# eora-ai/torchok

Measured on AMD Instinct MI355X. Metric: images/sec (node) ResNet-50 224px bs256/GPU; step p50 ms, higher is better.
Workload: dtype bf16

## Files before the change

### include/tok.h

```cpp
#ifndef TOK_H_
#define TOK_H_

#include <stddef.h>
#include <stdint.h>

#ifdef __cplusplus
extern "C" {
#endif

typedef enum tok_status {
  TOK_OK = 0,
  TOK_ERR_INVALID = -1,
  TOK_ERR_LAUNCH = -2,
  TOK_ERR_WORKSPACE = -3
} tok_status;

typedef enum tok_dtype { TOK_F32 = 0, TOK_F16 = 1, TOK_BF16 = 2 } tok_dtype;

typedef struct tok_conv_desc {
  int32_t n, h, w, c;
  int32_t k;
  int32_t r, s;
  int32_t p, q;
  int32_t stride, pad;
// ... 18 lines not shown

typedef struct tok_pack_item {
  const float* src;
  void* dst_fwd;
  void* dst_dgrad;
  int32_t k, r, s, c, k_pad, s_pad, c_pad;
  int32_t block_start;
} tok_pack_item;
int tok_pack_item_blocks(const tok_pack_item* item );
int tok_pack_weights_batched(const tok_pack_item* items_dev, int n_items, int total_blocks, void* stream);


int tok_conv_fwd_stat_rows(const tok_conv_desc* d);
int tok_conv_fwd(const tok_conv_desc* d, const void* x, const void* w, const float* bias,
                 void* y, float* stats, void* stream);
int tok_conv_dgrad(const tok_conv_desc* d, const void* dy, const void* w_dgrad, void* dx,
                   int accumulate, void* stream);
int tok_conv_dgrad_stat_rows(const tok_conv_desc* d);
int tok_conv_dgrad_bnstats(const tok_conv_desc* d, const void* dy, const void* w_dgrad, void* dx,
                           int accumulate, const void* bn_y, const uint8_t* bn_mask, float* partial,
                           void* stream);
typedef struct tok_bn_fused {
  int32_t* counters;
  int64_t count;
  int32_t c_real;
  int32_t param_accumulate;
  float momentum, eps;
  const float* gamma;
  const float* beta;
  float* running_mean;
  float* running_var;
  int64_t* nbt;
  float* mean;
  float* rstd;
  float* scale;
  float* shift;
  float* dgamma;
  float* dbeta;
  float* coef;
} tok_bn_fused;
int tok_conv_fwd_bn(const tok_conv_desc* d, const void* x, const void* w_fwd, void* y, float* stats,
                    const tok_bn_fused* bn, void* stream);
int tok_conv_dgrad_bn(const tok_conv_desc* d, const void* dy, const void* w_dgrad, void* dx, int accumulate,
                      const void* bn_y, const uint8_t* bn_mask, float* partial, const tok_bn_fused* bn,
                      void* stream);
int tok_bn_gram_finalize(const float* Z, const float* zsum, const float* w, int64_t count, int p, int k,
                         const float* gamma, const float* beta, float* running_mean, float* running_var,
                         int64_t* num_batches_tracked, float momentum, float eps, float* mean, float* rstd,
                         float* scale, float* shift, float* wz ,
                         void* stream);
int tok_conv_fwd_bn_apply(const tok_conv_desc* d, const void* x, const void* w, const float* scale, const float* shift,
                          const void* shortcut , int relu, void* out, uint8_t* mask ,
                          void* stream);
int tok_conv_dgrad_maskstore(const tok_conv_desc* d, const void* dy, const void* w_dgrad, void* dx, int accumulate,
                             const uint8_t* mask, float* partial, void* stream);
int tok_relu_mask_reduce(const void* dout, const uint8_t* mask, int64_t m, int c, void* dz, float* partial, void* stream);
int tok_bn3_bwd_prepare(const float* G, const float* w, const float* wz, const float* zsum, const float* partial, int rows,
                        int64_t count, int p, int k, const float* gamma, const float* mean, const float* rstd,
                        float* dgamma, float* dbeta, int param_accumulate, float* coef, float* dw, int dw_accumulate,
                        void* wa, void* wb, float* cvec, float* ws ,
                        void* stream);
size_t tok_bn3_bwd_prepare_ws_floats(int p, int k);
int tok_conv_dgrad_bias(const tok_conv_desc* d, const void* dy, const void* w_dgrad, const float* bias, void* dx,
                        int accumulate, const void* bn_y, const uint8_t* bn_mask, float* partial, void* stream);
int tok_subsample2_fwd(const void* x, int n, int h, int w, int c, void* out, void* stream);
int tok_subsample2_bwd(const void* dsub, int n, int h, int w, int c, void* dx, int accumulate, void* stream);
int tok_conv_dgrad_subacc_ok(const tok_conv_desc* d);
int tok_conv_dgrad_subacc(const tok_conv_desc* d, const void* dy, const void* w_dgrad, void* dx, const void* dsub,
                          const void* bn_y , const uint8_t* mask ,
                          float* partial , int mask_store, void* stream);
int tok_conv_dgrad2_ok(const tok_conv_desc* d1, const tok_conv_desc* d2);
int tok_conv_dgrad2(const tok_conv_desc* d1, const void* dy1, const void* w1_dgrad, const tok_conv_desc* d2, const void* dy2,
                    const void* w2_dgrad, const float* bias , void* dx, int accumulate,
                    const void* bn_y , const uint8_t* bn_mask , float* partial ,
                    void* stream);
size_t tok_conv_wgrad_ws_bytes(const tok_conv_desc* d);
int tok_conv_wgrad(const tok_conv_desc* d, const void* x, const void* dy, float* dw,
                   int k_real, int c_real, void* ws, size_t ws_bytes, int accumulate,
                   void* stream);
int tok_conv_wgrad_bias_ok(const tok_conv_desc* d);
size_t tok_conv_wgrad_bias_ws_bytes(const tok_conv_desc* d);
int tok_conv_wgrad_bias(const tok_conv_desc* d, const void* x, const void* dy, float* dw, int k_real, int c_real,
                        void* ws, size_t ws_bytes, int accumulate, float* dbias, int bias_accumulate, void* stream);


int tok_bn_finalize(const float* stats, int rows, int64_t count, int c, int c_real,
                    const float* gamma, const float* beta,
                    float* running_mean, float* running_var, int64_t* nbt,
                    float momentum, float eps,
                    float* mean, float* rstd, float* scale, float* shift, void* stream);
int tok_bn_eval_coeffs(const float* gamma, const float* beta, const float* running_mean,
                       const float* running_var, float eps, int c, int c_real,
                       float* scale, float* shift, void* stream);
int tok_bn_stats_rows(int64_t m, int c);
int tok_bn_stats(const void* y, int64_t m, int c, float* stats, void* stream);
int tok_bn_act_fwd(const void* y, const float* scale, const float* shift,
                   const void* shortcut, int relu, void* out, uint8_t* mask, int64_t m, int c,
                   void* stream);
void* tok_event_create(void);
int tok_event_destroy(void* ev);
int tok_next_launch_event(void* ev);
int tok_stream_wait_event(void* stream, void* ev);
int tok_bn_act_fwd_colsum_rows(int64_t m, int c);
int tok_bn_act_fwd_colsum(const void* y, const float* scale, const float* shift, const void* shortcut, int relu, void* out,
                          uint8_t* mask, int64_t m, int c, float* partial, void* stream);
int tok_bn_bwd_rows(int64_t m, int c);
int tok_bn_bwd_reduce(const void* dout, const void* y, const uint8_t* mask,
                      const float* scale, const float* shift,
                      const float* mean, const float* rstd, int relu,
                      int64_t m, int c, float* partial, void* stream);
int tok_bn_bwd_finalize(const float* partial, int rows, int64_t m, int c, int c_real,
                        const float* gamma, const float* mean, const float* rstd,
                        float* dgamma, float* dbeta, float* coef, int accumulate, int dzy_form,
                        void* stream);
int tok_bn_bwd_apply(const void* dout, const void* y, const uint8_t* mask,
                     const float* scale, const float* shift, const float* coef, int relu,
                     void* dy, void* dshortcut, int dshortcut_accumulate,
                     int64_t m, int c, void* stream);


int tok_maxpool3x3s2_fwd(const void* x, void* y, uint8_t* argmax, int n, int h, int w, int c,
                         void* stream);
int tok_maxpool3x3s2_bwd(const void* dy, const uint8_t* argmax, void* dx, int accumulate,
                         int n, int h, int w, int c, void* stream);
int tok_avgpool2x2_fwd(const void* x, void* y, int n, int h, int w, int c, void* stream);
int tok_avgpool2x2_bwd(const void* dy, void* dx, int accumulate, int n, int h, int w, int c, void* stream);
int tok_gap_fwd(const void* x, void* y, int n, int hw, int c, void* stream);
int tok_gap_bwd(const void* dy, void* dx, int accumulate, int n, int hw, int c, void* stream);
int tok_global_pool_fwd(const void* x, void* y, int* argmax, int n, int hw, int c, int ldy, int mode, void* stream);
int tok_global_pool_bwd(const void* dy, const int* argmax, void* dx, int accumulate, int n, int hw, int c, int ldy,
                        int mode, void* stream);

int tok_colsum(const void* dy, int64_t m, int n_pad, int n_real, float* out, int accumulate,
               void* stream);

#define TOK_CE_LOSS_FLOATS 2050
int tok_softmax_ce_fwd(const void* logits, const int64_t* target, int rows, int classes, int ld,
                       int64_t ignore_index, float* lse, float* row_loss,
                       float* loss , void* stream);
int tok_softmax_ce_bwd(const void* logits, const int64_t* target, const float* lse,
                       const float* loss, const float* gscale, int rows, int classes, int ld,
                       int64_t ignore_index, void* dlogits, void* stream);

int tok_softmax_ce_smooth_fwd(const void* logits, const int64_t* target, int rows, int classes, int ld,
                              int64_t ignore_index, float label_smoothing, float* lse, float* row_loss,
                              float* loss, void* stream);
int tok_softmax_ce_smooth_bwd(const void* logits, const int64_t* target, const float* lse, const float* loss,
                              const float* gscale, int rows, int classes, int ld, int64_t ignore_index,
                              float label_smoothing, void* dlogits, void* stream);

int tok_upsample_ce_serves(int classes, int ld);
int tok_upsample_ce_fwd(const void* low, int n, int hs, int ws, int classes, int ld, int hd, int wd, const int64_t* target,
                        int64_t ignore_index, float* lse, float* row_loss, float* loss, void* stream);
int tok_upsample_ce_bwd(const void* low, int n, int hs, int ws, int classes, int ld, int hd, int wd, const int64_t* target,
                        int64_t ignore_index, const float* lse, const float* loss, const float* gscale, void* dlow,
                        int accumulate, void* stream);

int tok_dice_rows(int64_t rows);
int tok_dice_fwd(const void* logits, const void* target, int64_t rows, int classes, int ld, int mode, float smooth,
                 float eps, int log_loss, const int64_t* class_sel, int n_sel, float* partial, float* loss,
                 float* coef, void* stream);
int tok_dice_bwd(const void* logits, const void* target, const float* coef, const float* gscale, int64_t rows,
                 int classes, int ld, int mode, void* dlogits, void* stream);

int tok_bce_logits_fwd(const void* logits, const float* target, int64_t rows, int classes, int ld,
                       float ignore_value, int mean, float* loss, void* stream);
// ... 215 lines not shown
```

### torchok_amd/_C.py

```python
import ctypes
import os
from ctypes import POINTER, Structure, c_char_p, c_float, c_int, c_int32, c_int64, c_size_t, c_void_p

_HERE = os.path.dirname(os.path.abspath(__file__))
LIB_PATH = os.environ.get('TOK_LIB') or os.path.join(_HERE, 'lib', 'libtok_gfx950.so')

TOK_F32, TOK_F16, TOK_BF16 = 0, 1, 2
TOK_CE_LOSS_FLOATS = 2050


class ConvDesc(Structure):
    _fields_ = [('n', c_int32), ('h', c_int32), ('w', c_int32), ('c', c_int32),
                ('k', c_int32), ('r', c_int32), ('s', c_int32),
                ('p', c_int32), ('q', c_int32),
                ('stride', c_int32), ('pad', c_int32), ('s_pad', c_int32)]


class PackItem(Structure):
    _fields_ = [('src', c_void_p), ('dst_fwd', c_void_p), ('dst_dgrad', c_void_p),
                ('k', c_int32), ('r', c_int32), ('s', c_int32), ('c', c_int32),
                ('k_pad', c_int32), ('s_pad', c_int32), ('c_pad', c_int32), ('block_start', c_int32)]


class BnFused(Structure):
    _fields_ = [('counters', c_void_p), ('count', c_int64), ('c_real', c_int32), ('param_accumulate', c_int32),
                ('momentum', c_float), ('eps', c_float), ('gamma', c_void_p), ('beta', c_void_p),
                ('running_mean', c_void_p), ('running_var', c_void_p), ('nbt', c_void_p), ('mean', c_void_p),
                ('rstd', c_void_p), ('scale', c_void_p), ('shift', c_void_p), ('dgamma', c_void_p),
                ('dbeta', c_void_p), ('coef', c_void_p)]


TOK_GRAD_CLIP_MAX_PARTIALS = 1024

_P = c_void_p
_PD = POINTER(ConvDesc)

PROTOTYPES = {
    'tok_last_error': (c_char_p, []),
    'tok_version': (c_int, []),
    'tok_nchw_to_nhwc_bf16': (c_int, [_P, c_int, c_int, c_int, c_int, c_int, _P, c_int, _P]),
    'tok_cast_f32_bf16': (c_int, [_P, _P, c_size_t, _P]),
    'tok_cast_bf16_f32': (c_int, [_P, _P, c_float, c_size_t, _P]),
    'tok_pack_weight_fwd': (c_int, [_P, c_int, c_int, c_int, c_int, _P, c_int, c_int, c_int, _P]),
    'tok_pack_weight_dgrad': (c_int, [_P, c_int, c_int, c_int, c_int, _P, c_int, c_int, _P]),
    'tok_pack_weight_both': (c_int, [_P, c_int, c_int, c_int, c_int, _P, c_int, c_int, c_int, _P, _P]),
    'tok_pack_item_blocks': (c_int, [POINTER(PackItem)]),
    'tok_pack_weights_batched': (c_int, [_P, c_int, c_int, _P]),
    'tok_conv_fwd_stat_rows': (c_int, [_PD]),
    'tok_conv_fwd': (c_int, [_PD, _P, _P, _P, _P, _P, _P]),
    'tok_conv_dgrad': (c_int, [_PD, _P, _P, _P, c_int, _P]),
    'tok_conv_dgrad_stat_rows': (c_int, [_PD]),
    'tok_conv_dgrad_bnstats': (c_int, [_PD, _P, _P, _P, c_int, _P, _P, _P, _P]),
    'tok_conv_fwd_bn': (c_int, [_PD, _P, _P, _P, _P, POINTER(BnFused), _P]),
    'tok_conv_dgrad_bn': (c_int, [_PD, _P, _P, _P, c_int, _P, _P, _P, POINTER(BnFused), _P]),
    'tok_conv_wgrad_ws_bytes': (c_size_t, [_PD]),
    'tok_conv_wgrad': (c_int, [_PD, _P, _P, _P, c_int, c_int, _P, c_size_t, c_int, _P]),
    'tok_conv_wgrad_bias_ok': (c_int, [_PD]),
    'tok_conv_wgrad_bias_ws_bytes': (c_size_t, [_PD]),
    'tok_conv_wgrad_bias': (c_int, [_PD, _P, _P, _P, c_int, c_int, _P, c_size_t, c_int, _P, c_int, _P]),
    'tok_bn_finalize': (c_int, [_P, c_int, c_int64, c_int, c_int, _P, _P, _P, _P, _P, c_float, c_float,
                                _P, _P, _P, _P, _P]),
    'tok_bn_eval_coeffs': (c_int, [_P, _P, _P, _P, c_float, c_int, c_int, _P, _P, _P]),
    'tok_bn_stats_rows': (c_int, [c_int64, c_int]),
    'tok_bn_stats': (c_int, [_P, c_int64, c_int, _P, _P]),
    'tok_bn_act_fwd': (c_int, [_P, _P, _P, _P, c_int, _P, _P, c_int64, c_int, _P]),
    'tok_bn_act_fwd_colsum_rows': (c_int, [c_int64, c_int]),
    'tok_event_create': (_P, []),
    'tok_event_destroy': (c_int, [_P]),
    'tok_next_launch_event': (c_int, [_P]),
    'tok_stream_wait_event': (c_int, [_P, _P]),
    'tok_bn_act_fwd_colsum': (c_int, [_P, _P, _P, _P, c_int, _P, _P, c_int64, c_int, _P, _P]),
    'tok_bn_bwd_rows': (c_int, [c_int64, c_int]),
    'tok_bn_bwd_reduce': (c_int, [_P, _P, _P, _P, _P, _P, _P, c_int, c_int64, c_int, _P, _P]),
    'tok_bn_bwd_finalize': (c_int, [_P, c_int, c_int64, c_int, c_int, _P, _P, _P, _P, _P, _P, c_int, c_int, _P]),
    'tok_bn_bwd_apply': (c_int, [_P, _P, _P, _P, _P, _P, c_int, _P, _P, c_int, c_int64, c_int, _P]),
    'tok_maxpool3x3s2_fwd': (c_int, [_P, _P, _P, c_int, c_int, c_int, c_int, _P]),
    'tok_maxpool3x3s2_bwd': (c_int, [_P, _P, _P, c_int, c_int, c_int, c_int, c_int, _P]),
    'tok_avgpool2x2_fwd': (c_int, [_P, _P, c_int, c_int, c_int, c_int, _P]),
    'tok_avgpool2x2_bwd': (c_int, [_P, _P, c_int, c_int, c_int, c_int, c_int, _P]),
    'tok_gap_fwd': (c_int, [_P, _P, c_int, c_int, c_int, _P]),
    'tok_gap_bwd': (c_int, [_P, _P, c_int, c_int, c_int, c_int, _P]),
    'tok_global_pool_fwd': (c_int, [_P, _P, _P, c_int, c_int, c_int, c_int, c_int, _P]),
    'tok_global_pool_bwd': (c_int, [_P, _P, _P, c_int, c_int, c_int, c_int, c_int, c_int, _P]),
    'tok_colsum': (c_int, [_P, c_int64, c_int, c_int, _P, c_int, _P]),
    'tok_bn_gram_finalize': (c_int, [_P, _P, _P, c_int64, c_int, c_int, _P, _P, _P, _P, _P, c_float, c_float, _P, _P, _P, _P, _P, _P]),
    'tok_conv_fwd_bn_apply': (c_int, [POINTER(ConvDesc), _P, _P, _P, _P, _P, c_int, _P, _P, _P]),
    'tok_conv_dgrad_maskstore': (c_int, [POINTER(ConvDesc), _P, _P, _P, c_int, _P, _P, _P]),
    'tok_relu_mask_reduce': (c_int, [_P, _P, c_int64, c_int, _P, _P, _P]),
    'tok_bn3_bwd_prepare': (c_int, [_P, _P, _P, _P, _P, c_int, c_int64, c_int, c_int, _P, _P, _P, _P, _P, c_int, _P, _P, c_int,
                                    _P, _P, _P, _P, _P]),
    'tok_bn3_bwd_prepare_ws_floats': (c_size_t, [c_int, c_int]),
    'tok_conv_dgrad_bias': (c_int, [POINTER(ConvDesc), _P, _P, _P, _P, c_int, _P, _P, _P, _P]),
    'tok_conv_dgrad2_ok': (c_int, [POINTER(ConvDesc), POINTER(ConvDesc)]),
    'tok_conv_dgrad2': (c_int, [POINTER(ConvDesc), _P, _P, POINTER(ConvDesc), _P, _P, _P, _P, c_int, _P, _P, _P, _P]),
    'tok_subsample2_fwd': (c_int, [_P, c_int, c_int, c_int, c_int, _P, _P]),
    'tok_subsample2_bwd': (c_int, [_P, c_int, c_int, c_int, c_int, _P, c_int, _P]),
    'tok_conv_dgrad_subacc_ok': (c_int, [POINTER(ConvDesc)]),
    'tok_conv_dgrad_subacc': (c_int, [POINTER(ConvDesc), _P, _P, _P, _P, _P, _P, _P, c_int, _P]),
    'tok_softmax_ce_fwd': (c_int, [_P, _P, c_int, c_int, c_int, c_int64, _P, _P, _P, _P]),
    'tok_softmax_ce_bwd': (c_int, [_P, _P, _P, _P, _P, c_int, c_int, c_int, c_int64, _P, _P]),
    'tok_softmax_ce_smooth_fwd': (c_int, [_P, _P, c_int, c_int, c_int, c_int64, c_float, _P, _P, _P, _P]),
    'tok_softmax_ce_smooth_bwd': (c_int, [_P, _P, _P, _P, _P, c_int, c_int, c_int, c_int64, c_float, _P, _P]),
    'tok_upsample_ce_serves': (c_int, [c_int, c_int]),
    'tok_upsample_ce_fwd': (c_int, [_P, c_int, c_int, c_int, c_int, c_int, c_int, c_int, _P, c_int64, _P, _P, _P, _P]),
    'tok_upsample_ce_bwd': (c_int, [_P, c_int, c_int, c_int, c_int, c_int, c_int, c_int, _P, c_int64, _P, _P, _P, _P, c_int, _P]),
    'tok_dice_rows': (c_int, [c_int64]),
    'tok_dice_fwd': (c_int, [_P, _P, c_int64, c_int, c_int, c_int, c_float, c_float, c_int, _P, c_int, _P, _P, _P, _P]),
    'tok_dice_bwd': (c_int, [_P, _P, _P, _P, c_int64, c_int, c_int, c_int, _P, _P]),
    'tok_bce_logits_fwd': (c_int, [_P, _P, c_int64, c_int, c_int, c_float, c_int, _P, _P]),
    'tok_bce_logits_bwd': (c_int, [_P, _P, _P, _P, c_int64, c_int, c_int, c_float, c_int, _P, _P]),
    'tok_relevance_matrix_multilabel': (c_int, [_P, _P, c_int, c_int, c_int, _P, _P]),
    'tok_embed_reg_fwd': (c_int, [_P, c_int, c_int, c_int, c_int, _P, _P, _P]),
    'tok_embed_reg_bwd': (c_int, [_P, _P, _P, c_float, c_int, c_int, c_int, c_int, _P, _P]),
    'tok_regression_loss_fwd': (c_int, [_P, _P, c_int64, c_int, c_float, c_int, _P, _P]),
    'tok_regression_loss_bwd': (c_int, [_P, _P, _P, c_int64, c_int, c_float, c_int, _P, _P]),
    'tok_confusion_update': (c_int, [_P, _P, _P, c_int64, c_int, c_int, c_int64, _P, _P]),
    'tok_cls_stats_update': (c_int, [_P, _P, _P, c_int64, c_int, c_int, c_int64, _P, _P]),
    'tok_l2norm_fwd': (c_int, [_P, _P, _P, c_int, c_int, c_int, c_int, c_float, _P]),
    'tok_l2norm_bwd': (c_int, [_P, _P, _P, _P, c_int, c_int, c_int, c_int, c_int, _P]),
    'tok_arcface_margin_fwd': (c_int, [_P, _P, c_int, c_int, c_int, c_float, c_float, c_float, c_float, c_int, c_float, _P, _P]),
    'tok_arcface_margin_bwd': (c_int, [_P, _P, _P, c_int, c_int, c_int, c_float, c_float, c_float, c_float, c_int, c_float, _P, _P]),
    'tok_relevance_matrix': (c_int, [_P, _P, c_int, c_int, _P, _P]),
    'tok_contrastive_fwd': (c_int, [_P, _P, _P, c_int, c_int, c_int, c_int, c_float, _P, _P, _P, _P]),
    'tok_contrastive_bwd': (c_int, [_P, _P, _P, _P, _P, c_int, c_int, c_int, c_int, c_float, _P, _P, c_int, _P]),
    'tok_fuse_sum_relu_fwd': (c_int, [_P, c_int, _P, c_int, _P, c_int, _P, c_int, c_int, c_int, c_int, c_int, c_int, _P, _P, _P]),
    'tok_fuse_sum_affine_relu_fwd': (c_int, [_P, c_int, _P, _P, _P, c_int, _P, _P, _P, c_int, _P, _P, _P, c_int, _P, _P, c_int, c_int, c_int, c_int, c_int, _P, _P, _P]),
    'tok_fuse_sum_relu_bwd': (c_int, [_P, _P, c_int, c_int, c_int, c_int, c_int, _P, c_int, _P]),
    'tok_bilinear_fwd': (c_int, [_P, c_int, c_int, c_int, c_int, c_int, _P, c_int, c_int, c_int, c_int, _P]),
    'tok_bilinear_bwd': (c_int, [_P, c_int, c_int, c_int, c_int, c_int, _P, c_int, c_int, c_int, c_int, c_int, _P]),
    'tok_bilinear_bwd_multi': (c_int, [_P, c_int, c_int, c_int, c_int, _P, c_int, c_int, _P, c_int, c_int, _P, c_int, c_int, _P]),
    'tok_bilinear_sum_stats_rows': (c_int, [c_int, c_int, c_int, c_int]),
    'tok_bilinear_sum_stats': (c_int, [_P, _P, c_int, c_int, _P, c_int, c_int, _P, c_int, c_int, c_int, c_int, c_int, c_int, _P, _P, _P]),
    'tok_layernorm_fwd': (c_int, [_P, _P, _P, c_int, _P, _P, _P, _P, _P, c_int64, c_int, c_int, c_float, _P]),
    'tok_layernorm_bwd_rows': (c_int, [c_int64, c_int]),
    'tok_layernorm_bwd': (c_int, [_P, _P, _P, _P, _P, _P, c_int, _P, c_int, _P, c_int64, c_int, c_int, _P]),
    'tok_colsum_partial_rows': (c_int, [c_int64, c_int]),
    'tok_colsum_partial': (c_int, [_P, c_int64, c_int, _P, _P]),
    'tok_colsum_f32': (c_int, [_P, c_int64, c_int, _P, c_int, _P]),
    'tok_colsum_f32_pair': (c_int, [_P, _P, c_int64, c_int, _P, c_int, _P, c_int, _P]),
    'tok_act_fwd': (c_int, [c_int, _P, _P, c_size_t, _P]),
    'tok_act_bwd': (c_int, [c_int, _P, _P, _P, c_int, c_size_t, _P]),
    'tok_window_attn_fwd': (c_int, [_P, c_int, c_int, c_int, c_int, c_int, c_int, c_int, c_int, _P, _P, _P, _P, _P, _P]),
# ... 105 lines not shown
```

### torchok_amd/csrc/bn.hip

```cpp
#include "tok_common.h"
#include <hip/hip_ext.h>
#include <stdlib.h>

static thread_local hipEvent_t t_done_event = nullptr;

namespace {

struct Geo {
  int cg_total, cge, rpb;
};
inline Geo make_geo(int c) {
  Geo g;
  g.cg_total = c / 8;
  g.cge = g.cg_total < 256 ? g.cg_total : 256;
  g.rpb = 256 / g.cge;
  return g;
}
inline int stream_blocks(int64_t m, const Geo& g, int cap) {
  int64_t b = (m + g.rpb - 1) / g.rpb;
  if (b > cap) b = cap;
  if (b < 1) b = 1;
  return (int)b;
}

// ... 250 lines not shown
        if (relu && mask != nullptr) {
          const unsigned bits = mask[(size_t)m * cg_total + cg];
#pragma unroll
          for (int e = 0; e < 8; ++e) {
            const float yf = bf2f(v[e]);
            const float dz = ((bits >> e) & 1u) ? bf2f(g[e]) : 0.f;
            s1[e] += dz;
            s2[e] = fmaf(dz, (yf - mu[e]) * rs[e], s2[e]);
          }
        } else {
#pragma unroll
          for (int e = 0; e < 8; ++e) {
            const float yf = bf2f(v[e]);
            float dz = bf2f(g[e]);
            if (relu && !(fmaf(yf, sc[e], sh[e]) > 0.f)) dz = 0.f;
            s1[e] += dz;
            s2[e] = fmaf(dz, (yf - mu[e]) * rs[e], s2[e]);
          }
        }
      }
    }
#pragma unroll
    for (int e = 0; e < 8; ++e) { red[0][tid][e] = s1[e]; red[1][tid][e] = s2[e]; }
    __syncthreads();
    if (rl == 0) {
      for (int r = 1; r < rpb; ++r)
#pragma unroll
        for (int e = 0; e < 8; ++e) { s1[e] += red[0][r * cge + cgl][e]; s2[e] += red[1][r * cge + cgl][e]; }
#pragma unroll
      for (int e = 0; e < 8; ++e) {
        partial[((size_t)0 * gridDim.x + blockIdx.x) * C + cg * 8 + e] = s1[e];
        partial[((size_t)1 * gridDim.x + blockIdx.x) * C + cg * 8 + e] = s2[e];
      }
    }
    __syncthreads();
  }
}

template <int CW>
__global__ __launch_bounds__(256) void bn_bwd_finalize_kernel(
    const float* __restrict__ partial, int rows, double inv_m, int C, int Creal, const float* __restrict__ gamma,
    const float* __restrict__ mean, const float* __restrict__ rstd, float* dgamma, float* dbeta,
    float* coef, int accumulate, int dzy_form) {
  __shared__ double red[2][256];
  constexpr int RL = 256 / CW;
  const int tid = threadIdx.x;
  const int cl = tid % CW, rl = tid / CW;
  const int c = blockIdx.x * CW + cl;
  double a1 = 0.0, a2 = 0.0;
  const bool owner = rl == 0 && c < Creal;
  float g_c = 0.f, mu_c = 0.f, rs_c = 0.f, dg_c = 0.f, db_c = 0.f;
  if (owner) {
    g_c = gamma[c]; mu_c = mean[c]; rs_c = rstd[c];
    if (accumulate && dgamma != nullptr) dg_c = dgamma[c];
    if (accumulate && dbeta != nullptr) db_c = dbeta[c];
  }
  if (c < C) {
    fold_rows<RL>(partial, rows, C, c, rl, a1, a2);
  }
  red[0][tid] = a1;
  red[1][tid] = a2;
  __syncthreads();
  for (int s = RL / 2; s > 0; s >>= 1) {
    if (rl < s) {
      red[0][tid] += red[0][tid + s * CW];
      red[1][tid] += red[1][tid + s * CW];
    }
    __syncthreads();
  }
  if (rl == 0 && c >= Creal && c < C) {
    coef[c] = 0.f; coef[C + c] = 0.f; coef[2 * C + c] = 0.f;
  }
  if (owner) {
    float sdz, sdzx, c1, c2, c3;
    bn_bwd_coeffs(red[0][tid], red[1][tid], dzy_form, inv_m, g_c, mu_c, rs_c, sdz, sdzx, c1, c2, c3);
    if (dgamma != nullptr) dgamma[c] = accumulate ? dg_c + sdzx : sdzx;
    if (dbeta != nullptr) dbeta[c] = accumulate ? db_c + sdz : sdz;
    coef[c] = c1;
    coef[C + c] = c2;
    coef[2 * C + c] = c3;
  }
}

__global__ __launch_bounds__(256) void bn_bwd_apply_kernel(
    const bf16* dout, const bf16* __restrict__ y, const uint8_t* __restrict__ mask,
    const float* __restrict__ scale, const float* __restrict__ shift, const float* __restrict__ coef,
    int relu, bf16* __restrict__ dy, bf16* dshortcut, int ds_acc, int64_t M, int C, int cge, int rpb) {
  const int tid = threadIdx.x;
  const int cgl = tid % cge, rl = tid / cge;
  if (rl >= rpb) return;
  const int cg_total = C >> 3;
  for (int cg = cgl; cg < cg_total; cg += cge) {
    float sc[8], sh[8], c1[8], c2[8], c3[8];
    load8f(scale + cg * 8, sc);
    load8f(shift + cg * 8, sh);
    load8f(coef + cg * 8, c1);
    load8f(coef + C + cg * 8, c2);
    load8f(coef + 2 * C + cg * 8, c3);
    for (int64_t m = (int64_t)blockIdx.x * rpb + rl; m < M; m += (int64_t)gridDim.x * rpb) {
      const size_t off = (size_t)m * C + cg * 8;
      const bf16x8 g = ldg16(dout + off);
      const bf16x8 v = ldg16(y + off);
      float dz[8];
      if (relu && mask != nullptr) {
        const unsigned bits = mask[(size_t)m * cg_total + cg];
#pragma unroll
        for (int e = 0; e < 8; ++e) dz[e] = ((bits >> e) & 1u) ? bf2f(g[e]) : 0.f;
      } else {
#pragma unroll
        for (int e = 0; e < 8; ++e) {
          dz[e] = bf2f(g[e]);
          if (relu && !(fmaf(bf2f(v[e]), sc[e], sh[e]) > 0.f)) dz[e] = 0.f;
        }
      }
      bf16x8 o;
#pragma unroll
      for (int e = 0; e < 8; ++e) o[e] = f2bf(fmaf(c1[e], dz[e], fmaf(c2[e], bf2f(v[e]), c3[e])));
      stg16(dy + off, o);
      if (dshortcut != nullptr) {
        bf16x8 d;
        if (ds_acc) {
          const bf16x8 old = ldg16(dshortcut + off);
#pragma unroll
          for (int e = 0; e < 8; ++e) d[e] = f2bf(dz[e] + bf2f(old[e]));
        } else {
#pragma unroll
          for (int e = 0; e < 8; ++e) d[e] = f2bf(dz[e]);
        }
        stg16(dshortcut + off, d);
      }
    }
  }
}



__global__ __launch_bounds__(256) void bn_relu_maxpool_fwd_kernel(const bf16* __restrict__ y,
                                                                  const float* __restrict__ scale,
                                                                  const float* __restrict__ shift, bf16* __restrict__ out,
                                                                  uint8_t* __restrict__ argmax, bf16* __restrict__ ypool,
                                                                  int N, int H, int W, int C, int P, int Q) {
  const int cg_total = C >> 3;
  const size_t total = (size_t)N * P * Q * cg_total;
  for (size_t i = (size_t)blockIdx.x * blockDim.x + threadIdx.x; i < total; i += (size_t)gridDim.x * blockDim.x) {
    const int cg = (int)(i % cg_total);
    size_t pix = i / cg_total;
    const int q = (int)(pix % Q);
    pix /= Q;
    const int p = (int)(pix % P);
    const int n = (int)(pix / P);
    float sc[8], sh[8];
    load8f(scale + cg * 8, sc);
    load8f(shift + cg * 8, sh);
    float best[8], ybest[8];
    int idx[8];
    bool first = true;
#pragma unroll
    for (int r = 0; r < 3; ++r) {
      const int h = 2 * p - 1 + r;
      if ((unsigned)h >= (unsigned)H) continue;
#pragma unroll
      for (int s = 0; s < 3; ++s) {
        const int w = 2 * q - 1 + s;
        if ((unsigned)w >= (unsigned)W) continue;
        const bf16x8 v = ldg16(y + (((size_t)n * H + h) * W + w) * C + cg * 8);
        if (first) {
#pragma unroll
          for (int e = 0; e < 8; ++e) { best[e] = -INFINITY; ybest[e] = 0.f; idx[e] = r * 3 + s; }
          first = false;
        }
#pragma unroll
        for (int e = 0; e < 8; ++e) {
          const float f = bf2f(f2bf(fmaxf(fmaf(bf2f(v[e]), sc[e], sh[e]), 0.f)));
          if (f > best[e] || f != f) { best[e] = f; ybest[e] = bf2f(v[e]); idx[e] = r * 3 + s; }
        }
      }
    }
    bf16x8 o;
    uint64_t packed = 0;
#pragma unroll
    for (int e = 0; e < 8; ++e) {
      o[e] = f2bf(best[e]);
      packed |= (uint64_t)(idx[e] & 0xff) << (8 * e);
    }
    const size_t off = (((size_t)n * P + p) * Q + q) * C + cg * 8;
    stg16(out + off, o);
    *reinterpret_cast<uint64_t*>(argmax + off) = packed;
    if (ypool != nullptr) {
      bf16x8 yo;
#pragma unroll
      for (int e = 0; e < 8; ++e) yo[e] = f2bf(ybest[e]);
      stg16(ypool + off, yo);
    }
  }
}

__device__ __forceinline__ void pooled_dz(const bf16* __restrict__ dpool, const uint8_t* __restrict__ argmax,
                                          const bf16x8 yv, const float (&sc)[8], const float (&sh)[8], int n, int h,
                                          int w, int C, int P, int Q, int cg, float (&dz)[8]) {
  float g[8];
#pragma unroll
  for (int e = 0; e < 8; ++e) g[e] = 0.f;
  const int p0 = h >> 1, p1 = (h + 1) >> 1, q0 = w >> 1, q1 = (w + 1) >> 1;
  const bool vp[2] = {p0 < P, p1 != p0 && p1 < P}, vq[2] = {q0 < Q, q1 != q0 && q1 < Q};
  const int pc[2] = {p0 < P ? p0 : P - 1, vp[1] ? p1 : (p0 < P ? p0 : P - 1)};
  const int qc[2] = {q0 < Q ? q0 : Q - 1, vq[1] ? q1 : (q0 < Q ? q0 : Q - 1)};
  uint64_t packed[4];
  bf16x8 d[4];
#pragma unroll
  for (int a = 0; a < 2; ++a)
#pragma unroll
    for (int b = 0; b < 2; ++b) {
// ... 355 lines not shown
```

### torchok_amd/csrc/conv_wgrad.hip

```cpp
#include "tok_common.h"
#include "conv_common.h"
#include <type_traits>
#include <stdlib.h>

namespace {

struct WgradArgs {
  const bf16* x;
  const bf16* dy;
  float* ws;
  int H, W, C, K, R, S, P, Q, stride, pad;
  int M, PQ, HW, Ktot;
  int tilesN, tilesK, splitM, mchunk;
  uint32_t x_bytes, dy_bytes;
  uint32_t pq_mul, pq_shift, q_mul, q_shift;
  float* cs;
  int cs_cols;
  int adv_q, adv_p;
  size_t cs_stride, ws_stride;
};

__device__ __forceinline__ uint32_t magic_div(uint32_t n, uint32_t mul, uint32_t shift) {
  return (uint32_t)(((uint64_t)__umulhi(n, mul) + n) >> shift);
}
// ... 898 lines not shown
    asm volatile("s_waitcnt vmcnt(%0) lgkmcnt(0)" ::"n"((NST - 2) * LOADS) : "memory");
    __builtin_amdgcn_s_barrier();
    __builtin_amdgcn_sched_barrier(0);
    const int rd2 = rd == NST - 1 ? 0 : rd + 1;
    bf16x8 af[NT];
#pragma unroll
    for (int i = 0; i < NT; ++i) af[i] = __builtin_bit_cast(bf16x8, (u32x4){ycur[i][0][0], ycur[i][0][1], ycur[i][1][0], ycur[i][1][1]});
#pragma unroll
    for (int j = 0; j < KTL; ++j) {
      if (W0 * KTL + j < NTILES) {
        const bf16x8 bfr = __builtin_bit_cast(bf16x8, (u32x4){xb[j][0][0], xb[j][0][1], xb[j][1][0], xb[j][1][1]});
#pragma unroll
        for (int i = 0; i < NT; ++i) acc[i][j] = __builtin_amdgcn_mfma_f32_16x16x32_bf16(af[i], bfr, acc[i][j], 0, 0, 0);
      }
      if (j < LOADS) issue_piece(wr, j);
      if (j == 0) advance();
      if (j >= 1 && (j - 1) * 2 < NT) { read_y(rd, (j - 1) * 2, ynxt); if ((j - 1) * 2 + 1 < NT) read_y(rd, (j - 1) * 2 + 1, ynxt); }
      read_x(tb, j, xb);
#pragma unroll
      for (int k = 0; k < 3; ++k)
        if (last_j(k) == j) bases_tap(rd2, k, tb);
      __builtin_amdgcn_sched_barrier(0);
    }
    rd = rd2;
    wr = wr == NST - 1 ? 0 : wr + 1;
  };
  for (int st = 0; st < steps; st += 2) {
    body(yA, yB);
    if (st + 1 < steps) body(yB, yA);
  }
  asm volatile("s_waitcnt vmcnt(0) lgkmcnt(0)" ::: "memory");

  int lane2;
  asm volatile("v_mbcnt_lo_u32_b32 %0, -1, 0\n\tv_mbcnt_hi_u32_b32 %0, -1, %0" : "=v"(lane2));
  const int g = lane2 >> 4, li = lane2 & 15;
  float* out = a.ws + (size_t)split * a.K * a.Ktot;
#pragma unroll
  for (int j = 0; j < KTL; ++j) {
    const int J = W0 * KTL + j;
    if (J >= NTILES) continue;
    const int cin = ct * TC + (J % CT) * 16 + li;
    const int kcol = (J / CT) * a.C + cin;
#pragma unroll
    for (int i = 0; i < NT; ++i)
#pragma unroll
      for (int r = 0; r < 4; ++r) {
        const int n = tn * TN + i * 16 + g * 4 + r;
        if (n < a.K && cin < a.C) out[(size_t)n * a.Ktot + kcol] = acc[i][j][r];
      }
  }
  };
  if (wv == 0) run(std::integral_constant<int, 0>{});
  else if (wv == 1) run(std::integral_constant<int, 1>{});
  else if (wv == 2) run(std::integral_constant<int, 2>{});
  else run(std::integral_constant<int, 3>{});
}

__global__ void wgrad_reduce_kernel(const float* __restrict__ ws, float* __restrict__ dw, int splitM,
                                    int k_real, int R, int S, int c_real, int K, int S_pad,
                                    int C_pad, int accumulate) {
  const size_t total = (size_t)k_real * R * S * c_real;
  const size_t slab = (size_t)K * R * S_pad * C_pad;
  for (size_t i = (size_t)blockIdx.x * blockDim.x + threadIdx.x; i < total;
       i += (size_t)gridDim.x * blockDim.x) {
    const int c = (int)(i % c_real);
    size_t rest = i / c_real;
    const int s = (int)(rest % S);
    rest /= S;
    const int r = (int)(rest % R);
    const int k = (int)(rest / R);
    const size_t src = (((size_t)k * R + r) * S_pad + s) * C_pad + c;
    float t = 0.f;
    for (int sp = 0; sp < splitM; sp += 8) {
      float v[8];
#pragma unroll
      for (int u = 0; u < 8; ++u) v[u] = ws[(size_t)(sp + u < splitM ? sp + u : splitM - 1) * slab + src];
#pragma unroll
      for (int u = 0; u < 8; ++u) t += sp + u < splitM ? v[u] : 0.f;
    }
    dw[i] = accumulate ? dw[i] + t : t;
  }
}

template <int U>
__device__ __forceinline__ void reduce_slabs(const float* __restrict__ ws, size_t stride, size_t i, int row, int splitM, float4& t) {
  for (int sp = row; sp < splitM; sp += 16 * U) {
    float4 v[U];
#pragma unroll
    for (int u = 0; u < U; ++u) {
      const int su = sp + 16 * u;
      v[u] = reinterpret_cast<const float4*>(ws + (size_t)(su < splitM ? su : splitM - 1) * stride)[i];
    }
#pragma unroll
    for (int u = 0; u < U; ++u) {
      if (sp + 16 * u < splitM) { t.x += v[u].x; t.y += v[u].y; t.z += v[u].z; t.w += v[u].w; }
    }
  }
}

__global__ __launch_bounds__(256) void wgrad_reduce_flat_kernel(const float* __restrict__ ws, float* __restrict__ dw,
                                                                int splitM, size_t slab, int accumulate, size_t stride,
                                                                float* __restrict__ extra, int extra_n, int extra_pad,
                                                                int extra_acc) {
  __shared__ float4 red[16][16];
  const int col = threadIdx.x & 15, row = threadIdx.x >> 4;
  const size_t m4 = slab >> 2;
  const size_t n4 = m4 + (extra != nullptr ? (size_t)(extra_pad >> 2) : 0);
  for (size_t base = (size_t)blockIdx.x * 16; base < n4; base += (size_t)gridDim.x * 16) {
    const size_t i = base + col;
    float4 t = {0.f, 0.f, 0.f, 0.f};
    if (i < n4) {
      if (splitM > 64) reduce_slabs<8>(ws, stride, i, row, splitM, t);
      else if (splitM > 32) reduce_slabs<4>(ws, stride, i, row, splitM, t);
      else if (splitM > 16) reduce_slabs<2>(ws, stride, i, row, splitM, t);
      else if (row < splitM) {
        const float4 v = reinterpret_cast<const float4*>(ws + (size_t)row * stride)[i];
        t.x += v.x; t.y += v.y; t.z += v.z; t.w += v.w;
      }
    }
    red[row][col] = t;
    __syncthreads();
    for (int s_ = 8; s_ > 0; s_ >>= 1) {
      if (row < s_) {
        const float4 o = red[row + s_][col];
        float4 m = red[row][col];
        m.x += o.x; m.y += o.y; m.z += o.z; m.w += o.w;
        red[row][col] = m;
      }
      __syncthreads();
    }
    if (row == 0 && i < m4) {
      float4 r = red[0][col];
      if (accumulate) {
        const float4 o = reinterpret_cast<const float4*>(dw)[i];
        r.x += o.x; r.y += o.y; r.z += o.z; r.w += o.w;
      }
      reinterpret_cast<float4*>(dw)[i] = r;
    } else if (row == 0 && i < n4) {
      const float4 r = red[0][col];
      const float rv[4] = {r.x, r.y, r.z, r.w};
      const int e0 = (int)(i - m4) * 4;
#pragma unroll
      for (int e = 0; e < 4; ++e)
        if (e0 + e < extra_n) extra[e0 + e] = extra_acc ? extra[e0 + e] + rv[e] : rv[e];
    }
    __syncthreads();
  }
}

struct Plan {
  int TN, TK, tilesN, tilesK, splitM, mchunk, MS;
  bool ring;
  bool taps;
};

static int taps_enabled() {
  static const int v = [] { const char* e = getenv("TOK_WGRAD_TAPS"); return (int)(e ? atoi(e) : 1); }();
  return v;
}
static int taps_target() {
  static const int v = [] { const char* e = getenv("TOK_WGRAD_TAPS_WGS"); return (int)(e ? atoi(e) : 256); }();
  return v;
}

static int ring_enabled() {
  static const int v = [] { const char* e = getenv("TOK_WGRAD_RING"); return (int)(e ? atoi(e) : 1); }();
  return v;
}
static int ring_target() {
  static const int v = [] { const char* e = getenv("TOK_WGRAD_WGS"); return (int)(e ? atoi(e) : 0); }();
  return v;
}

Plan make_plan(const tok_conv_desc* d) {
  Plan p;
  const int Ktot = d->r * d->s_pad * d->c;
  const long long M = (long long)d->n * d->p * d->q;
  p.taps = false;
  const bool same3 = d->r == 3 && d->s == 3 && d->s_pad == 3 && d->stride == 1 && d->pad == 1 && taps_enabled() != 2 &&
                     (unsigned long long)d->n * d->h * d->w * d->c * 2 < 0x40000000ull &&
                     (unsigned long long)d->n * d->p * d->q * d->k * 2 < 0x40000000ull;
  const bool w64 = d->c % 64 == 0 && d->k % 64 == 0;
  const bool w48 = !w64 && d->c % 48 == 0 && d->k % 48 == 0 && same3 && taps_enabled() != 3;
  if (d->c != 4 && (w64 || w48) && d->r == 3 && d->s == 3 && d->s_pad == 3 && taps_enabled()) {
    p.taps = true; p.ring = false;
    p.TN = w64 ? 64 : 48; p.TK = p.TN; p.MS = 32;
    p.tilesN = tok_cdiv(d->k, p.TN);
    p.tilesK = tok_cdiv(d->c, p.TN);
    const int tiles = p.tilesN * p.tilesK;
    long long split = (taps_target() + tiles - 1) / tiles;
    const long long max_split = (M + 8 * 32 - 1) / (8 * 32);
    if (split > max_split) split = max_split;
    if (split > 512) split = 512;
    if (split < 1) split = 1;
    long long chunk = (M + split - 1) / split;
    chunk = ((chunk + 31) / 32) * 32;
    p.mchunk = (int)chunk;
    p.splitM = (int)((M + chunk - 1) / chunk);
    return p;
  }
  p.ring = d->c != 4 && ring_enabled() && ((d->r == 1 && d->s == 1 && d->stride == 1 && d->pad == 0) || ring_enabled() == 2);
  if (p.ring) {
    p.MS = 32;
    if (d->k <= 64) { p.TN = 64; p.TK = Ktot >= 256 ? 256 : (Ktot >= 128 ? 128 : 64); }
    else if (Ktot <= 64) { p.TK = 64; p.TN = d->k >= 256 ? 256 : 128; }
    else { p.TN = 128; p.TK = 128; }
    static const int big = [] { const char* e = getenv("TOK_WGRAD_256"); return (int)(e ? atoi(e) : 1); }();
    if (big && d->r == 1 && d->s == 1 && d->stride == 1 && d->pad == 0 && d->k >= 256 && Ktot >= 256 && M >= (big >= 2 ? 8192 : 200000) &&
        (long long)tok_cdiv(d->k, 256) * tok_cdiv(Ktot, 256) * 65536 * 2 <= (long long)d->k * Ktot * 3) {
      p.TN = 256; p.TK = 256;
    }
    p.tilesN = tok_cdiv(d->k, p.TN);
    p.tilesK = tok_cdiv(Ktot, p.TK);
    const int tiles = p.tilesN * p.tilesK;
    const int stage = 32 * (p.TN + p.TK) * 2;
    const int per_cu = (160 * 1024) / (3 * stage);
    static const int long_target = [] { const char* e = getenv("TOK_WGRAD_WGS_LONG"); return (int)(e ? atoi(e) : 0); }();
    const int target = (long_target > 0 && M >= 100000) ? long_target
                       : ring_target() > 0 ? ring_target() : 256 * (per_cu > 2 ? 2 : per_cu);
    long long split = (target + tiles - 1) / tiles;
    const long long max_split = (M + 8 * 32 - 1) / (8 * 32);
    if (split > max_split) split = max_split;
    if (split > 512) split = 512;
    if (split < 1) split = 1;
    long long chunk = (M + split - 1) / split;
    chunk = ((chunk + 31) / 32) * 32;
    p.mchunk = (int)chunk;
    p.splitM = (int)((M + chunk - 1) / chunk);
    return p;
  }
// ... 133 lines not shown
  a.stride = d->stride; a.pad = d->pad;
  a.M = d->n * d->p * d->q; a.PQ = d->p * d->q; a.HW = d->h * d->w;
  make_magic((uint32_t)a.PQ, a.pq_mul, a.pq_shift);
  make_magic((uint32_t)d->q, a.q_mul, a.q_shift);
  a.adv_q = 32 % d->q; a.adv_p = (32 / d->q) % d->p;
  a.Ktot = d->r * d->s_pad * d->c;
  a.tilesN = p.tilesN; a.tilesK = p.tilesK; a.splitM = p.splitM; a.mchunk = p.mchunk;
  const size_t slab_f = (size_t)d->k * d->r * d->s_pad * d->c;
  const int cs_pad = (k_real + 3) / 4 * 4;
  const bool cs_inline = dbias != nullptr && flat && !direct;
  a.ws_stride = cs_inline ? slab_f + cs_pad : slab_f;
  a.cs = dbias ? (cs_inline ? (float*)ws + slab_f : (float*)((char*)ws + tok_conv_wgrad_ws_bytes(d))) : nullptr;
  a.cs_stride = cs_inline ? a.ws_stride : (size_t)k_real;
  a.cs_cols = k_real;
  {
    const unsigned long long xb = (unsigned long long)d->n * d->h * d->w * d->c * 2;
    const unsigned long long yb = (unsigned long long)a.M * d->k * 2;
    TOK_CHECK_ARG(xb < 0xFFFFFFF0ull && yb < 0xFFFFFFF0ull, "tok_conv_wgrad: tensors of 4 GiB or more are not supported");
    a.x_bytes = (uint32_t)xb; a.dy_bytes = (uint32_t)yb;
  }
  hipStream_t st = tok_stream(stream);
  const bool c4 = d->c == 4;
  if (c4 && dbias == nullptr && stem_wgrad_serves(d)) {
    stem_wgrad_launch(d, x, dy, a.ws, p.splitM, st);
  } else
  if (p.taps) {
    constexpr int smem = 3 * 10 * 32 * 128;
    static const bool attr_set = [&] {
      (void)hipFuncSetAttribute(reinterpret_cast<const void*>(&conv_wgrad_taps_kernel<0>),
                                hipFuncAttributeMaxDynamicSharedMemorySize, smem);
      return true;
    }();
    (void)attr_set;
    const bool same = a.stride == 1 && a.pad == 1 && a.P == a.H && a.Q == a.W && a.x_bytes < 0x40000000u && a.dy_bytes < 0x40000000u &&
                      taps_enabled() != 2;
    if (same) {
      constexpr int smem_p = 3 * (32 * 128 + 128 * 128);
      static const bool attr_p = [&] {
        (void)hipFuncSetAttribute(reinterpret_cast<const void*>(&conv_wgrad_winp_kernel<4, 3, 9>), hipFuncAttributeMaxDynamicSharedMemorySize, smem_p);
        (void)hipFuncSetAttribute(reinterpret_cast<const void*>(&conv_wgrad_winp_kernel<3, 3, 7>), hipFuncAttributeMaxDynamicSharedMemorySize, smem_p);
        return true;
      }();
      (void)attr_p;
      const dim3 gw(a.tilesN * a.tilesK * a.splitM);
      if (p.TN == 48) hipLaunchKernelGGL((conv_wgrad_winp_kernel<3, 3, 7>), gw, dim3(256), smem_p, st, a);
      else hipLaunchKernelGGL((conv_wgrad_winp_kernel<4, 3, 9>), gw, dim3(256), smem_p, st, a);
    } else {
      hipLaunchKernelGGL((conv_wgrad_taps_kernel<0>), dim3(a.tilesN * a.tilesK * a.splitM), dim3(256), smem, st, a);
    }
  } else if (p.ring) {
    if (p.TN == 256 && p.TK == 256) {
      constexpr int smem8 = 3 * 32 * (256 + 256) * 2;
      static const bool attr8 = [] {
        (void)hipFuncSetAttribute(reinterpret_cast<const void*>(&conv_wgrad_ring8_kernel<256, 256>),
                                  hipFuncAttributeMaxDynamicSharedMemorySize, smem8);
        return true;
      }();
      (void)attr8;
      hipLaunchKernelGGL((conv_wgrad_ring8_kernel<256, 256>), dim3(a.tilesN * a.tilesK * a.splitM), dim3(512), smem8, st, a);
    }
    else if (p.TN == 64 && p.TK == 64) launch_ring<64, 64>(a, st);
    else if (p.TN == 64 && p.TK == 128) launch_ring<64, 128>(a, st);
    else if (p.TN == 64 && p.TK == 256) launch_ring<64, 256>(a, st);
    else if (p.TN == 128 && p.TK == 64) launch_ring<128, 64>(a, st);
    else if (p.TN == 256 && p.TK == 64) launch_ring<256, 64>(a, st);
    else launch_ring<128, 128>(a, st);
  } else if (p.TN == 128 && p.TK == 128) {
    if (c4) launch_wgrad<128, 128, true>(a, st, p.MS); else launch_wgrad<128, 128, false>(a, st, p.MS);
  } else if (p.TN == 128) {
    if (c4) launch_wgrad<128, 64, true>(a, st, p.MS); else launch_wgrad<128, 64, false>(a, st, p.MS);
  } else if (p.TK == 128) {
    if (c4) launch_wgrad<64, 128, true>(a, st, p.MS); else launch_wgrad<64, 128, false>(a, st, p.MS);
  } else {
    if (c4) launch_wgrad<64, 64, true>(a, st, p.MS); else launch_wgrad<64, 64, false>(a, st, p.MS);
  }
  TOK_CHECK_LAUNCH("tok_conv_wgrad");
  if (dbias != nullptr && !cs_inline) {
    if (int e = tok_colsum_f32(a.cs, p.splitM, k_real, dbias, bias_accumulate, stream)) return e;
  }
  if (direct) return TOK_OK;
  if (flat) {
    if (tok_dbg_skip(2)) return TOK_OK;
    const size_t slab = (size_t)d->k * d->r * d->s * d->c;
    const size_t nb = (slab / 4 + 15) / 16;
    hipLaunchKernelGGL(wgrad_reduce_flat_kernel, dim3((int)(nb < 4096 ? nb : 4096)), dim3(256), 0, st,
                       (const float*)ws, dw, p.splitM, slab, accumulate, cs_inline ? a.ws_stride : slab,
                       cs_inline ? dbias : (float*)nullptr, k_real, cs_inline ? cs_pad : 0, bias_accumulate);
    TOK_CHECK_LAUNCH("tok_conv_wgrad(reduce)");
    return TOK_OK;
  }
  const size_t total = (size_t)k_real * d->r * d->s * c_real;
  const int blocks = (int)((total + 255) / 256 < 2048 ? (total + 255) / 256 : 2048);
  hipLaunchKernelGGL(wgrad_reduce_kernel, dim3(blocks), dim3(256), 0, st, (const float*)ws, dw,
                     p.splitM, k_real, d->r, d->s, c_real, d->k, d->s_pad, d->c, accumulate);
  TOK_CHECK_LAUNCH("tok_conv_wgrad(reduce)");
  return TOK_OK;
}
}
```

Baseline: 14630.

## Rewrite wgrad split reduction as wave-shuffle kernel and batch BN bwd apply rows

```diff
diff --git a/include/tok.h b/include/tok.h
--- a/include/tok.h
+++ b/include/tok.h
@@ -124,6 +124,8 @@
 size_t tok_conv_wgrad_bias_ws_bytes(const tok_conv_desc* d);
 int tok_conv_wgrad_bias(const tok_conv_desc* d, const void* x, const void* dy, float* dw, int k_real, int c_real,
                         void* ws, size_t ws_bytes, int accumulate, float* dbias, int bias_accumulate, void* stream);
+int tok_wgrad_reduce_flat(const float* ws, float* dw, int split_m, size_t slab, int accumulate, size_t stride, float* extra,
+                          int extra_n, int extra_pad, int extra_acc, void* stream);
 
 
 int tok_bn_finalize(const float* stats, int rows, int64_t count, int c, int c_real,
diff --git a/torchok_amd/_C.py b/torchok_amd/_C.py
--- a/torchok_amd/_C.py
+++ b/torchok_amd/_C.py
@@ -58,6 +58,7 @@
     'tok_conv_wgrad_bias_ok': (c_int, [_PD]),
     'tok_conv_wgrad_bias_ws_bytes': (c_size_t, [_PD]),
     'tok_conv_wgrad_bias': (c_int, [_PD, _P, _P, _P, c_int, c_int, _P, c_size_t, c_int, _P, c_int, _P]),
+    'tok_wgrad_reduce_flat': (c_int, [_P, _P, c_int, c_size_t, c_int, c_size_t, _P, c_int, c_int, c_int, _P]),
     'tok_bn_finalize': (c_int, [_P, c_int, c_int64, c_int, c_int, _P, _P, _P, _P, _P, c_float, c_float,
                                 _P, _P, _P, _P, _P]),
     'tok_bn_eval_coeffs': (c_int, [_P, _P, _P, _P, c_float, c_int, c_int, _P, _P, _P]),
diff --git a/torchok_amd/csrc/bn.hip b/torchok_amd/csrc/bn.hip
--- a/torchok_amd/csrc/bn.hip
+++ b/torchok_amd/csrc/bn.hip
@@ -356,6 +356,7 @@
   }
 }
 
+constexpr int APPLY_ROWS = 2;
 __global__ __launch_bounds__(256) void bn_bwd_apply_kernel(
     const bf16* dout, const bf16* __restrict__ y, const uint8_t* __restrict__ mask,
     const float* __restrict__ scale, const float* __restrict__ shift, const float* __restrict__ coef,
@@ -364,6 +365,8 @@
   const int cgl = tid % cge, rl = tid / cge;
   if (rl >= rpb) return;
   const int cg_total = C >> 3;
+  const bool use_mask = relu && mask != nullptr, read_old = dshortcut != nullptr && ds_acc;
+  const int64_t step = (int64_t)gridDim.x * rpb;
   for (int cg = cgl; cg < cg_total; cg += cge) {
     float sc[8], sh[8], c1[8], c2[8], c3[8];
     load8f(scale + cg * 8, sc);
@@ -371,37 +374,51 @@
     load8f(coef + cg * 8, c1);
     load8f(coef + C + cg * 8, c2);
     load8f(coef + 2 * C + cg * 8, c3);
-    for (int64_t m = (int64_t)blockIdx.x * rpb + rl; m < M; m += (int64_t)gridDim.x * rpb) {
-      const size_t off = (size_t)m * C + cg * 8;
-      const bf16x8 g = ldg16(dout + off);
-      const bf16x8 v = ldg16(y + off);
-      float dz[8];
-      if (relu && mask != nullptr) {
-        const unsigned bits = mask[(size_t)m * cg_total + cg];
-#pragma unroll
-        for (int e = 0; e < 8; ++e) dz[e] = ((bits >> e) & 1u) ? bf2f(g[e]) : 0.f;
-      } else {
-#pragma unroll
-        for (int e = 0; e < 8; ++e) {
-          dz[e] = bf2f(g[e]);
-          if (relu && !(fmaf(bf2f(v[e]), sc[e], sh[e]) > 0.f)) dz[e] = 0.f;
-        }
-      }
-      bf16x8 o;
-#pragma unroll
-      for (int e = 0; e < 8; ++e) o[e] = f2bf(fmaf(c1[e], dz[e], fmaf(c2[e], bf2f(v[e]), c3[e])));
-      stg16(dy + off, o);
-      if (dshortcut != nullptr) {
-        bf16x8 d;
-        if (ds_acc) {
-          const bf16x8 old = ldg16(dshortcut + off);
-#pragma unroll
-          for (int e = 0; e < 8; ++e) d[e] = f2bf(dz[e] + bf2f(old[e]));
+    for (int64_t m0 = (int64_t)blockIdx.x * rpb + rl; m0 < M; m0 += APPLY_ROWS * step) {
+      bf16x8 g[APPLY_ROWS], v[APPLY_ROWS], old[APPLY_ROWS];
+      unsigned bits[APPLY_ROWS];
+#pragma unroll
+      for (int r = 0; r < APPLY_ROWS; ++r) {
+        const int64_t m = m0 + r * step;
+        if (m < M) {
+          const size_t off = (size_t)m * C + cg * 8;
+          g[r] = ldg16(dout + off);
+          v[r] = ldg16(y + off);
+          if (use_mask) bits[r] = mask[(size_t)m * cg_total + cg];
+          if (read_old) old[r] = ldg16(dshortcut + off);
+        }
+      }
+#pragma unroll
+      for (int r = 0; r < APPLY_ROWS; ++r) {
+        const int64_t m = m0 + r * step;
+        if (m >= M) break;
+        const size_t off = (size_t)m * C + cg * 8;
+        float dz[8];
+        if (use_mask) {
+#pragma unroll
+          for (int e = 0; e < 8; ++e) dz[e] = ((bits[r] >> e) & 1u) ? bf2f(g[r][e]) : 0.f;
         } else {
 #pragma unroll
-          for (int e = 0; e < 8; ++e) d[e] = f2bf(dz[e]);
-        }
-        stg16(dshortcut + off, d);
+          for (int e = 0; e < 8; ++e) {
+            dz[e] = bf2f(g[r][e]);
+            if (relu && !(fmaf(bf2f(v[r][e]), sc[e], sh[e]) > 0.f)) dz[e] = 0.f;
+          }
+        }
+        bf16x8 o;
+#pragma unroll
+        for (int e = 0; e < 8; ++e) o[e] = f2bf(fmaf(c1[e], dz[e], fmaf(c2[e], bf2f(v[r][e]), c3[e])));
+        stg16(dy + off, o);
+        if (dshortcut != nullptr) {
+          bf16x8 d;
+          if (read_old) {
+#pragma unroll
+            for (int e = 0; e < 8; ++e) d[e] = f2bf(dz[e] + bf2f(old[r][e]));
+          } else {
+#pragma unroll
+            for (int e = 0; e < 8; ++e) d[e] = f2bf(dz[e]);
+          }
+          stg16(dshortcut + off, d);
+        }
       }
     }
   }
diff --git a/torchok_amd/csrc/conv_wgrad.hip b/torchok_amd/csrc/conv_wgrad.hip
--- a/torchok_amd/csrc/conv_wgrad.hip
+++ b/torchok_amd/csrc/conv_wgrad.hip
@@ -1004,70 +1004,99 @@
   }
 }
 
-template <int U>
-__device__ __forceinline__ void reduce_slabs(const float* __restrict__ ws, size_t stride, size_t i, int row, int splitM, float4& t) {
-  for (int sp = row; sp < splitM; sp += 16 * U) {
-    float4 v[U];
-#pragma unroll
-    for (int u = 0; u < U; ++u) {
-      const int su = sp + 16 * u;
-      v[u] = reinterpret_cast<const float4*>(ws + (size_t)(su < splitM ? su : splitM - 1) * stride)[i];
-    }
-#pragma unroll
-    for (int u = 0; u < U; ++u) {
-      if (sp + 16 * u < splitM) { t.x += v[u].x; t.y += v[u].y; t.z += v[u].z; t.w += v[u].w; }
-    }
-  }
-}
-
+__device__ __forceinline__ void add4(float4& t, const float4& v) { t.x += v.x; t.y += v.y; t.z += v.z; t.w += v.w; }
+
+template <int G>
 __global__ __launch_bounds__(256) void wgrad_reduce_flat_kernel(const float* __restrict__ ws, float* __restrict__ dw,
                                                                 int splitM, size_t slab, int accumulate, size_t stride,
                                                                 float* __restrict__ extra, int extra_n, int extra_pad,
                                                                 int extra_acc) {
-  __shared__ float4 red[16][16];
-  const int col = threadIdx.x & 15, row = threadIdx.x >> 4;
+  constexpr int L = 16 / G, CPW = 64 / L, D = 16 / G;
+  const int lane = threadIdx.x & 63, lr = lane % L, cw = lane / L;
   const size_t m4 = slab >> 2;
   const size_t n4 = m4 + (extra != nullptr ? (size_t)(extra_pad >> 2) : 0);
-  for (size_t base = (size_t)blockIdx.x * 16; base < n4; base += (size_t)gridDim.x * 16) {
-    const size_t i = base + col;
-    float4 t = {0.f, 0.f, 0.f, 0.f};
+  const size_t wave = (size_t)blockIdx.x * 4 + (threadIdx.x >> 6), nwaves = (size_t)gridDim.x * 4;
+  for (size_t base = wave * CPW; base < n4; base += nwaves * CPW) {
+    const size_t i = base + cw;
+    float4 p[G];
+#pragma unroll
+    for (int j = 0; j < G; ++j) p[j] = make_float4(0.f, 0.f, 0.f, 0.f);
     if (i < n4) {
-      if (splitM > 64) reduce_slabs<8>(ws, stride, i, row, splitM, t);
-      else if (splitM > 32) reduce_slabs<4>(ws, stride, i, row, splitM, t);
-      else if (splitM > 16) reduce_slabs<2>(ws, stride, i, row, splitM, t);
-      else if (row < splitM) {
-        const float4 v = reinterpret_cast<const float4*>(ws + (size_t)row * stride)[i];
-        t.x += v.x; t.y += v.y; t.z += v.z; t.w += v.w;
-      }
-    }
-    red[row][col] = t;
-    __syncthreads();
-    for (int s_ = 8; s_ > 0; s_ >>= 1) {
-      if (row < s_) {
-        const float4 o = red[row + s_][col];
-        float4 m = red[row][col];
-        m.x += o.x; m.y += o.y; m.z += o.z; m.w += o.w;
-        red[row][col] = m;
-      }
-      __syncthreads();
-    }
-    if (row == 0 && i < m4) {
-      float4 r = red[0][col];
-      if (accumulate) {
-        const float4 o = reinterpret_cast<const float4*>(dw)[i];
-        r.x += o.x; r.y += o.y; r.z += o.z; r.w += o.w;
-      }
+      const float4* src = reinterpret_cast<const float4*>(ws) + i;
+      const size_t s4 = stride >> 2;
+      for (int k0 = 0; k0 * 16 < splitM; k0 += D) {
+        float4 v[D][G];
+#pragma unroll
+        for (int d = 0; d < D; ++d)
+#pragma unroll
+          for (int j = 0; j < G; ++j) {
+            const int s = lr + L * j + 16 * (k0 + d);
+            if (s < splitM) v[d][j] = src[(size_t)s * s4];
+          }
+#pragma unroll
+        for (int d = 0; d < D; ++d)
+#pragma unroll
+          for (int j = 0; j < G; ++j)
+            if (lr + L * j + 16 * (k0 + d) < splitM) add4(p[j], v[d][j]);
+      }
+    }
+#pragma unroll
+    for (int h = G / 2; h >= 1; h >>= 1)
+#pragma unroll
+      for (int j = 0; j < h; ++j) add4(p[j], p[j + h]);
+#pragma unroll
+    for (int h = L / 2; h >= 1; h >>= 1) {
+      float4 o;
+      o.x = __shfl_down(p[0].x, h); o.y = __shfl_down(p[0].y, h);
+      o.z = __shfl_down(p[0].z, h); o.w = __shfl_down(p[0].w, h);
+      if (lr < h) add4(p[0], o);
+    }
+    if (lr == 0 && i < m4) {
+      float4 r = p[0];
+      if (accumulate) add4(r, reinterpret_cast<const float4*>(dw)[i]);
       reinterpret_cast<float4*>(dw)[i] = r;
-    } else if (row == 0 && i < n4) {
-      const float4 r = red[0][col];
-      const float rv[4] = {r.x, r.y, r.z, r.w};
+    } else if (lr == 0 && i < n4) {
+      const float rv[4] = {p[0].x, p[0].y, p[0].z, p[0].w};
       const int e0 = (int)(i - m4) * 4;
 #pragma unroll
       for (int e = 0; e < 4; ++e)
         if (e0 + e < extra_n) extra[e0 + e] = extra_acc ? extra[e0 + e] + rv[e] : rv[e];
     }
-    __syncthreads();
-  }
+  }
+}
+
+int reduce_rows_per_thread(int splitM) {
+  const int per_chain = (splitM + 15) / 16;
+  int g = 16;
+  while (g > 1 && g * per_chain > 16) g >>= 1;
+  return g;
+}
+
+int launch_reduce_flat(const float* ws, float* dw, int splitM, size_t slab, int accumulate, size_t stride, float* extra,
+                       int extra_n, int extra_pad, int extra_acc, hipStream_t st) {
+  static const int cus = [] {
+    int dev = 0, n = 0;
+    if (hipGetDevice(&dev) != hipSuccess || hipDeviceGetAttribute(&n, hipDeviceAttributeMultiprocessorCount, dev) != hipSuccess || n < 1) n = 256;
+    return n;
+  }();
+  const int G = reduce_rows_per_thread(splitM);
+  const size_t n4 = slab / 4 + (extra != nullptr ? (size_t)(extra_pad / 4) : 0);
+  const size_t cols_per_block = 4 * (size_t)(64 / (16 / G));
+  size_t nb = (n4 + cols_per_block - 1) / cols_per_block;
+  const size_t cap = (size_t)cus * 8;
+  if (nb > cap) nb = cap;
+  if (nb < 1) nb = 1;
+#define TOK_REDUCE_FLAT(g_) hipLaunchKernelGGL(wgrad_reduce_flat_kernel<g_>, dim3((unsigned)nb), dim3(256), 0, st, ws, dw, splitM, \
+                                               slab, accumulate, stride, extra, extra_n, extra_pad, extra_acc)
+  switch (G) {
+    case 16: TOK_REDUCE_FLAT(16); break;
+    case 8: TOK_REDUCE_FLAT(8); break;
+    case 4: TOK_REDUCE_FLAT(4); break;
+    case 2: TOK_REDUCE_FLAT(2); break;
+    default: TOK_REDUCE_FLAT(1); break;
+  }
+#undef TOK_REDUCE_FLAT
+  return TOK_OK;
 }
 
 struct Plan {
@@ -1367,10 +1396,8 @@
   if (flat) {
     if (tok_dbg_skip(2)) return TOK_OK;
     const size_t slab = (size_t)d->k * d->r * d->s * d->c;
-    const size_t nb = (slab / 4 + 15) / 16;
-    hipLaunchKernelGGL(wgrad_reduce_flat_kernel, dim3((int)(nb < 4096 ? nb : 4096)), dim3(256), 0, st,
-                       (const float*)ws, dw, p.splitM, slab, accumulate, cs_inline ? a.ws_stride : slab,
-                       cs_inline ? dbias : (float*)nullptr, k_real, cs_inline ? cs_pad : 0, bias_accumulate);
+    launch_reduce_flat((const float*)ws, dw, p.splitM, slab, accumulate, cs_inline ? a.ws_stride : slab,
+                       cs_inline ? dbias : (float*)nullptr, k_real, cs_inline ? cs_pad : 0, bias_accumulate, st);
     TOK_CHECK_LAUNCH("tok_conv_wgrad(reduce)");
     return TOK_OK;
   }
@@ -1382,3 +1409,15 @@
   return TOK_OK;
 }
 }
+
+extern "C" int tok_wgrad_reduce_flat(const float* ws, float* dw, int split_m, size_t slab, int accumulate, size_t stride,
+                                     float* extra, int extra_n, int extra_pad, int extra_acc, void* stream) {
+  TOK_CHECK_ARG(ws && dw && split_m >= 1 && slab > 0 && slab % 4 == 0 && stride % 4 == 0 && stride >= slab,
+                "tok_wgrad_reduce_flat: bad arguments");
+  TOK_CHECK_ARG(((uintptr_t)ws & 15) == 0 && ((uintptr_t)dw & 15) == 0, "tok_wgrad_reduce_flat: unaligned buffers");
+  TOK_CHECK_ARG(extra == nullptr || (extra_pad % 4 == 0 && extra_n <= extra_pad && slab + extra_pad <= stride),
+                "tok_wgrad_reduce_flat: bad extra vector");
+  launch_reduce_flat(ws, dw, split_m, slab, accumulate, stride, extra, extra_n, extra ? extra_pad : 0, extra_acc, tok_stream(stream));
+  TOK_CHECK_LAUNCH("tok_wgrad_reduce_flat");
+  return TOK_OK;
+}
```

After: 14760 (median of 6 runs). No clear change (+0.8%).
